# TaiseiNiman/SimpleGaussianSplat_tk71

Measured on AMD Instinct MI355X. Metric: splat-pixel pairs blended per second (grouped cumprod fwd+bwd), higher is better.
Workload: dtype f32; 1 GPU; cfg3: 1920x1080, 1000000 Gaussians, mean 80 splats/pixel (deep heavy-tailed lists); pairs_per_gpu=166335639, pixel_groups_per_gpu=2073600, bytes_per_pair=32, tiles_left_to_the_follow_up_kernel=0, world_size_checked=1, tiles_resolved_through_the_descriptor_tree=1258

## Files before the change

simplegaussiansplat_tk71_amd/csrc/gcp_bin.hip:

```cpp

#include <hip/hip_runtime.h>
#include <stdint.h>

#include "gcp_tiles.hpp"

namespace {
using namespace gcp;

constexpr int kScanChunk = 2048;

__device__ __forceinline__ int block_excl_scan_256(int v, int* s_w, int& total) {
  const int lane = threadIdx.x & 63, w = threadIdx.x >> 6;
  const int inc = wave_incl_scan_i(v);
  if (lane == 63) s_w[w] = inc;
  __syncthreads();
  int woff = 0, tot = 0;
#pragma unroll
  for (int j = 0; j < 4; ++j) { const int t = s_w[j]; if (j < w) woff += t; tot += t; }
  total = tot;
  __syncthreads();
  return woff + inc - v;
}

__global__ __launch_bounds__(256) void k_scan_reduce(const int* in, int* bsum, i64 n) {
  __shared__ int s_w[4];
  const i64 base = (i64)blockIdx.x * kScanChunk + (i64)threadIdx.x * 8;
  int s = 0;
#pragma unroll
  for (int k = 0; k < 8; ++k) if (base + k < n) s += in[base + k];
  int total;
  block_excl_scan_256(s, s_w, total);
  if (threadIdx.x == 0) bsum[blockIdx.x] = total;
}

__global__ __launch_bounds__(256) void k_scan_apply(const int* in, const int* bsum, int* out, i64 n, i64 nb) {
  __shared__ int s_w[4];
  int part = 0;
  for (i64 j = threadIdx.x; j < (i64)blockIdx.x; j += 256) part += bsum[j];
  int boff;
  block_excl_scan_256(part, s_w, boff);
  const i64 base = (i64)blockIdx.x * kScanChunk + (i64)threadIdx.x * 8;
  int v[8];
  int s = 0;
#pragma unroll
  for (int k = 0; k < 8; ++k) { v[k] = (base + k < n) ? in[base + k] : 0; s += v[k]; }
  int total;
  int ex = block_excl_scan_256(s, s_w, total) + boff;
#pragma unroll
  for (int k = 0; k < 8; ++k) { if (base + k < n) out[base + k] = ex; ex += v[k]; }
  if ((i64)blockIdx.x == nb - 1 && threadIdx.x == 0) out[n] = boff + total;
}

}

int gcp::launch_excl_scan(const int* in, int* out, i64 n, int* ws, hipStream_t stream) {
  if (n <= 0) {
    GCP_HIP(hipMemsetAsync(out, 0, sizeof(int), stream));
    return GCP_OK;
  }
  const i64 nb = (n + kScanChunk - 1) / kScanChunk;
  hipLaunchKernelGGL(k_scan_reduce, dim3((unsigned)nb), dim3(256), 0, stream, in, ws, n);
  hipLaunchKernelGGL(k_scan_apply, dim3((unsigned)nb), dim3(256), 0, stream, in, (const int*)ws, out, n, nb);
  GCP_HIP(hipGetLastError());
  return GCP_OK;
}

namespace {

__global__ __launch_bounds__(256) void k_tile_count(const int* start, const int* end, i64 n, int W, int H, int* cnt,
                                                     unsigned long long* total64) {
  __shared__ unsigned long long s_total;
  if (threadIdx.x == 0) s_total = 0;
  __syncthreads();
  unsigned long long wide = 0;
  for (i64 g = (i64)blockIdx.x * blockDim.x + threadIdx.x; g < n; g += (i64)gridDim.x * blockDim.x) {
    Box b;
    int c = 0;
    if (load_box(start, end, g, W, H, b))
      c = ((b.x1 >> kTileLog2) - (b.x0 >> kTileLog2) + 1) * ((b.y1 >> kTileLog2) - (b.y0 >> kTileLog2) + 1);
    cnt[g] = c;
    wide += (unsigned long long)c;
  }
  if (wide) atomicAdd(&s_total, wide);
  __syncthreads();
  if (threadIdx.x == 0 && s_total) atomicAdd(total64, s_total);
}

constexpr int kEmitWide = 128;
__global__ __launch_bounds__(256) void k_tile_emit(const int* start, const int* end, i64 n, int W, int H, int tiles_x,
                                                   const int* off, unsigned* key, unsigned* val, i64 capacity, int* info,
                                                   const unsigned long long* total64) {
  const i64 g = (i64)blockIdx.x * blockDim.x + threadIdx.x;
  const int lane = threadIdx.x & 63;
  bool live = g < n;
  if (info) {
    if (*total64 > 0x7fffffffull) {
      if (g == 0) { info[0] = 0; info[1] = 1; }
      return;
    }
    if (live) {
      const i64 lo = off[g], hi = off[g + 1];
      if (g == 0 && (i64)off[n] <= capacity) { info[0] = off[n]; info[1] = 0; }
      if (lo <= capacity && hi > capacity) { info[0] = (int)lo; info[1] = 1; }
      if (hi > capacity) live = false;
    }
  }
  Box b = {0, 0, -1, -1};
  if (live) live = load_box(start, end, g, W, H, b);
  const int tx0 = b.x0 >> kTileLog2, ty0 = b.y0 >> kTileLog2;
  const int ntx = live ? (b.x1 >> kTileLog2) - tx0 + 1 : 0, nty = live ? (b.y1 >> kTileLog2) - ty0 + 1 : 0;
  const int e0 = live ? off[g] : 0;
  const bool wide = ntx * nty >= kEmitWide;
  if (live && !wide) {
    int e = e0;
    for (int ty = ty0; ty < ty0 + nty; ++ty)
      for (int tx = tx0; tx < tx0 + ntx; ++tx) {
        key[e] = (unsigned)(ty * tiles_x + tx);
        val[e] = (unsigned)g;
        ++e;
      }
  }
  for (unsigned long long todo = __ballot(wide); todo; todo &= todo - 1ull) {
    const int owner = __builtin_ctzll(todo);
    const int wtx0 = __builtin_amdgcn_readlane(tx0, owner), wty0 = __builtin_amdgcn_readlane(ty0, owner);
    const int wntx = __builtin_amdgcn_readlane(ntx, owner), wcount = wntx * __builtin_amdgcn_readlane(nty, owner);
    const int we0 = __builtin_amdgcn_readlane(e0, owner);
    const unsigned wg = (unsigned)(g - lane + owner);
    for (int i = lane; i < wcount; i += 64) {
      const int ty = i / wntx, tx = i - ty * wntx;
      key[we0 + i] = (unsigned)((wty0 + ty) * tiles_x + wtx0 + tx);
      val[we0 + i] = wg;
    }
  }
}

__global__ __launch_bounds__(256) void k_sort_hist(const unsigned* key, i64 n, int shift, int* hist, int nblk, const int* n_dev,
                                                   int xcd_remap) {
  __shared__ int h[256];
  const i64 chunk = sort_chunk(blockIdx.x, nblk, xcd_remap);
  if (chunk < 0) return;
  if (n_dev) n = min(n, (i64)*n_dev);
  h[threadIdx.x] = 0;
  __syncthreads();
  const i64 base = chunk * kSortChunk;
#pragma unroll 4
  for (int i = threadIdx.x; i < kSortChunk; i += 256)
    if (base + i < n) atomicAdd(&h[(key[base + i] >> shift) & 255u], 1);
  __syncthreads();
  hist[(i64)threadIdx.x * nblk + chunk] = h[threadIdx.x];
}

__global__ __launch_bounds__(256) void k_sort_scatter(const unsigned* key, const unsigned* val, unsigned* key_out,
                                                       unsigned* val_out, i64 n, int shift, const int* hist_excl,
                                                       int nblk, const int* n_dev, int xcd_remap) {
  const i64 chunk = sort_chunk(blockIdx.x, nblk, xcd_remap);
  if (chunk < 0) return;
  if (n_dev) n = min(n, (i64)*n_dev);
  __shared__ unsigned s_key[kSortChunk];
  __shared__ unsigned s_val[kSortChunk];
  __shared__ int off[4][256];
  __shared__ int gdelta[256];
  __shared__ int s_w[4];
  const int tid = threadIdx.x, lane = tid & 63, w = tid >> 6;
  for (int d = lane; d < 256; d += 64) off[w][d] = 0;
  __syncthreads();
  const i64 bbase = chunk * kSortChunk;
  const i64 wbase = bbase + (i64)w * (kSortChunk / 4);
  constexpr int kSteps = kSortChunk / 4 / 64;
  unsigned k[kSteps], v[kSteps];
#pragma unroll
  for (int st = 0; st < kSteps; ++st) {
    const i64 i = wbase + st * 64 + lane;
    const bool valid = i < n;
    k[st] = valid ? key[i] : 0u;
    v[st] = valid ? val[i] : 0u;
    if (valid) atomicAdd(&off[w][(k[st] >> shift) & 255u], 1);
  }
  __syncthreads();
  {
    const int c0 = off[0][tid], c1 = off[1][tid], c2 = off[2][tid], c3 = off[3][tid];
    int total;
    const int lstart = block_excl_scan_256(c0 + c1 + c2 + c3, s_w, total);
    off[0][tid] = lstart;
    off[1][tid] = lstart + c0;
    off[2][tid] = lstart + c0 + c1;
    off[3][tid] = lstart + c0 + c1 + c2;
    gdelta[tid] = hist_excl[(i64)tid * nblk + chunk] - lstart;
  }
  __syncthreads();
#pragma unroll
  for (int st = 0; st < kSteps; ++st) {
    const i64 i = wbase + st * 64 + lane;
    const bool valid = i < n;
    const unsigned d = (k[st] >> shift) & 255u;
    unsigned long long peers = __ballot(valid);
#pragma unroll
    for (int b = 0; b < 8; ++b) {
      const bool bit = (d >> b) & 1u;
      const unsigned long long m = __ballot(bit);
      peers &= bit ? m : ~m;
    }
    const int rank = __builtin_popcountll(peers & ((1ull << lane) - 1ull));
    const int pos = off[w][d];
    if (valid && rank == 0) off[w][d] = pos + __builtin_popcountll(peers);
    if (valid) {
      s_key[pos + rank] = k[st];
      s_val[pos + rank] = v[st];
    }
  }
  __syncthreads();
  const int nvalid = (int)((n - bbase < kSortChunk) ? (n - bbase) : kSortChunk);
  for (int i = tid; i < nvalid; i += 256) {
    const unsigned kk = s_key[i];
    const i64 g = (i64)i + gdelta[(kk >> shift) & 255u];
    key_out[g] = kk;
    val_out[g] = s_val[i];
  }
}

__global__ void k_tile_bounds(const unsigned* key, i64 K, int n_tiles, int* tile_start, const int* n_dev) {
  if (n_dev) K = min(K, (i64)*n_dev);
  const i64 i = (i64)blockIdx.x * blockDim.x + threadIdx.x;
  if (i > K) return;
  const int prev = (i == 0) ? -1 : (int)key[i - 1];
  const int cur = (i == K) ? n_tiles : (int)key[i];
  for (int t = prev + 1; t <= cur; ++t) tile_start[t] = (int)i;
}

}

extern "C" {

int gcp_tile_grid(int32_t width, int32_t height, int32_t* tiles_x, int32_t* tiles_y) {
  if (width < 0 || height < 0 || !tiles_x || !tiles_y) return GCP_ERR_INVALID_ARGUMENT;
  const TileGrid t = tile_grid(width, height);
  *tiles_x = t.tx;
  *tiles_y = t.ty;
  return GCP_OK;
}

size_t gcp_scan_i32_workspace_bytes(int64_t n) {
  return align256((size_t)((n + kScanChunk - 1) / kScanChunk + 1) * sizeof(int));
}

int gcp_exclusive_scan_i32(const int32_t* in, int32_t* out, int64_t n, void* ws, size_t ws_bytes, void* stream) {
  if (n < 0 || !out || (n > 0 && (!in || !ws))) return GCP_ERR_INVALID_ARGUMENT;
  if (n > 0 && ws_bytes < gcp_scan_i32_workspace_bytes(n)) return GCP_ERR_WORKSPACE;
  return launch_excl_scan(in, out, n, (int*)ws, (hipStream_t)stream);
}

static int count_tiles(const int32_t* start_xy, const int32_t* end_xy, int64_t n_gauss, int32_t width, int32_t height,
                       int32_t* tile_off, unsigned long long* total64, void* ws, hipStream_t stream) {
  char* p = (char*)ws + 256;
  int* cnt = carve<int>(p, (size_t)n_gauss);
  int* sws = (int*)p;
  GCP_HIP(hipMemsetAsync(total64, 0, sizeof(unsigned long long), stream));
  const i64 count_blocks = (n_gauss + 255) / 256 < 512 ? (n_gauss + 255) / 256 : 512;
  hipLaunchKernelGGL(k_tile_count, dim3((unsigned)count_blocks), dim3(256), 0, stream, start_xy, end_xy,
                     (i64)n_gauss, width, height, cnt, total64);
  GCP_HIP(hipGetLastError());
  return launch_excl_scan(cnt, tile_off, n_gauss, sws, stream);
}

int gcp_bin_tiles_count(const int32_t* start_xy, const int32_t* end_xy, int64_t n_gauss, int32_t width,
                        int32_t height, int32_t* tile_off, int64_t* n_tile_pairs_host, void* ws,
                        size_t ws_bytes, void* stream_) {
  hipStream_t stream = (hipStream_t)stream_;
  if (n_gauss < 0 || width < 0 || height < 0 || !tile_off || !n_tile_pairs_host) return GCP_ERR_INVALID_ARGUMENT;
  *n_tile_pairs_host = 0;
  if (n_gauss == 0) {
    GCP_HIP(hipMemsetAsync(tile_off, 0, sizeof(int), stream));
    return GCP_OK;
  }
  if (!start_xy || !end_xy || !ws) return GCP_ERR_INVALID_ARGUMENT;
  const size_t need = 256 + align256((size_t)n_gauss * sizeof(int)) + gcp_scan_i32_workspace_bytes(n_gauss);
  if (ws_bytes < need) return GCP_ERR_WORKSPACE;
  unsigned long long* total64 = (unsigned long long*)ws;
  const int st = count_tiles(start_xy, end_xy, n_gauss, width, height, tile_off, total64, ws, stream);
  if (st != GCP_OK) return st;
  unsigned long long total = 0;
  GCP_HIP(hipMemcpyAsync(&total, total64, sizeof(total), hipMemcpyDeviceToHost, stream));
  GCP_HIP(hipStreamSynchronize(stream));
  if (total > 0x7fffffffull) return GCP_ERR_INVALID_ARGUMENT;
  *n_tile_pairs_host = (int64_t)total;
  return GCP_OK;
}

size_t gcp_bin_workspace_bytes(int64_t n_gauss, int64_t n_tile_pairs) {
  const int64_t k = n_tile_pairs > 0 ? n_tile_pairs : 1;
  const int64_t nblk = (k + kSortChunk - 1) / kSortChunk;
  size_t b = 0;
  b += 3 * align256((size_t)k * sizeof(unsigned));
  b += 2 * align256((size_t)(256 * nblk + 1) * sizeof(int));
  b += gcp_scan_i32_workspace_bytes(256 * nblk);
  const size_t count_need = 256 + align256((size_t)(n_gauss > 0 ? n_gauss : 1) * sizeof(int)) +
                            gcp_scan_i32_workspace_bytes(n_gauss > 0 ? n_gauss : 1);
  return (b > count_need ? b : count_need) + 512;
}

static int bin_fill(const int32_t* start_xy, const int32_t* end_xy, int64_t n_gauss, int32_t width, int32_t height,
                    const int32_t* tile_off, int64_t K, int32_t* tile_start, int32_t* tile_list, int* info,
                    const unsigned long long* total64, void* ws, hipStream_t stream) {
  const TileGrid tg = tile_grid(width, height);
  const int n_tiles = tg.tx * tg.ty;
  const i64 nblk = (K + kSortChunk - 1) / kSortChunk;
  char* p = (char*)ws;
  unsigned* keyA = carve<unsigned>(p, (size_t)K);
  unsigned* keyB = carve<unsigned>(p, (size_t)K);
  unsigned* valB = carve<unsigned>(p, (size_t)K);
  int* hist = carve<int>(p, (size_t)(256 * nblk + 1));
  int* hist_ex = carve<int>(p, (size_t)(256 * nblk + 1));
  int* sws = (int*)p;
  unsigned* valA = (unsigned*)tile_list;
  const int* n_dev = info;

  hipLaunchKernelGGL(k_tile_emit, dim3((unsigned)((n_gauss + 255) / 256)), dim3(256), 0, stream, start_xy, end_xy,
                     (i64)n_gauss, width, height, tg.tx, tile_off, keyA, valA, (i64)K, info, total64);
  GCP_HIP(hipGetLastError());
  int bits = 1;
  while ((1 << bits) < n_tiles) ++bits;
  int passes = (bits + 7) / 8;
  if (passes & 1) ++passes;
  unsigned *ks = keyA, *vs = valA, *kd = keyB, *vd = valB;
  for (int pass = 0; pass < passes; ++pass) {
    const int shift = 8 * pass;
    hipLaunchKernelGGL(k_sort_hist, dim3((unsigned)nblk), dim3(256), 0, stream, (const unsigned*)ks, K, shift, hist, (int)nblk, n_dev, 0);
    GCP_HIP(hipGetLastError());
    const int st = launch_excl_scan(hist, hist_ex, 256 * nblk, sws, stream);
    if (st != GCP_OK) return st;
    hipLaunchKernelGGL(k_sort_scatter, dim3((unsigned)nblk), dim3(256), 0, stream, (const unsigned*)ks,
                       (const unsigned*)vs, kd, vd, K, shift, (const int*)hist_ex, (int)nblk, n_dev, 0);
    GCP_HIP(hipGetLastError());
    unsigned* t;
    t = ks; ks = kd; kd = t;
    t = vs; vs = vd; vd = t;
  }
  hipLaunchKernelGGL(k_tile_bounds, dim3((unsigned)((K + 1 + 255) / 256)), dim3(256), 0, stream, ks, K, n_tiles,
                     tile_start, n_dev);
  GCP_HIP(hipGetLastError());
  return GCP_OK;
}

int gcp_bin_tiles_fill(const int32_t* start_xy, const int32_t* end_xy, int64_t n_gauss, int32_t width,
                       int32_t height, const int32_t* tile_off, int64_t n_tile_pairs, int32_t* tile_start,
                       int32_t* tile_list, void* ws, size_t ws_bytes, void* stream_) {
  hipStream_t stream = (hipStream_t)stream_;
  if (n_gauss < 0 || n_tile_pairs < 0 || width < 0 || height < 0 || !tile_start) return GCP_ERR_INVALID_ARGUMENT;
  const TileGrid tg = tile_grid(width, height);
  const int n_tiles = tg.tx * tg.ty;
  const i64 K = n_tile_pairs;
  if (K == 0) {
    GCP_HIP(hipMemsetAsync(tile_start, 0, (size_t)(n_tiles + 1) * sizeof(int), stream));
    return GCP_OK;
  }
  if (!start_xy || !end_xy || !tile_off || !tile_list || !ws) return GCP_ERR_INVALID_ARGUMENT;
  if (ws_bytes < gcp_bin_workspace_bytes(n_gauss, K)) return GCP_ERR_WORKSPACE;
  return bin_fill(start_xy, end_xy, n_gauss, width, height, tile_off, K, tile_start, tile_list, nullptr, nullptr, ws, stream);
}

int gcp_bin_tiles(const int32_t* start_xy, const int32_t* end_xy, int64_t n_gauss, int32_t width, int32_t height,
                  int64_t capacity, int32_t* tile_off, int32_t* tile_start, int32_t* tile_list, int32_t* info, void* ws,
                  size_t ws_bytes, void* stream_) {
  hipStream_t stream = (hipStream_t)stream_;
  if (n_gauss < 0 || width < 0 || height < 0 || capacity < 1 || capacity > 0x7fffffffLL || !tile_off || !tile_start || !tile_list ||
      !info || !ws)
    return GCP_ERR_INVALID_ARGUMENT;
  const TileGrid tg = tile_grid(width, height);
  const int n_tiles = tg.tx * tg.ty;
  if (n_gauss == 0) {
    GCP_HIP(hipMemsetAsync(tile_off, 0, sizeof(int), stream));
    GCP_HIP(hipMemsetAsync(tile_start, 0, (size_t)(n_tiles + 1) * sizeof(int), stream));
    GCP_HIP(hipMemsetAsync(info, 0, 2 * sizeof(int), stream));
    return GCP_OK;
  }
  if (!start_xy || !end_xy) return GCP_ERR_INVALID_ARGUMENT;
  if (ws_bytes < gcp_bin_workspace_bytes(n_gauss, capacity)) return GCP_ERR_WORKSPACE;
  unsigned long long* total64 = (unsigned long long*)((char*)ws + ((ws_bytes - 256) & ~(size_t)255));
  const int st = count_tiles(start_xy, end_xy, n_gauss, width, height, tile_off, total64, ws, stream);
  if (st != GCP_OK) return st;
  return bin_fill(start_xy, end_xy, n_gauss, width, height, tile_off, capacity, tile_start, tile_list, info, total64, ws, stream);
}

}
```

simplegaussiansplat_tk71_amd/csrc/gcp_sort.hip:

```cpp

#include <hip/hip_runtime.h>
#include <stdint.h>

#include "gcp_tiles.hpp"

namespace {
using namespace gcp;

constexpr int kBigChunk = 4096;
constexpr int kSortSub = 8;

__device__ __forceinline__ void count_runs(int* h, unsigned d, int lane) {
  const unsigned dl = (unsigned)dpp_i<0x138, 0xf>((int)0xffffffffu, (int)d);
  const bool head = (lane == 0) || (d != dl);
  const unsigned long long heads = __ballot(head);
  if (head && d < 256u) {
    const unsigned long long above = (lane == 63) ? 0ull : (heads >> (lane + 1));
    const int len = above ? (__builtin_ctzll(above) + 1) : (64 - lane);
    atomicAdd(&h[d], len);
  }
}

struct SortPass { int shift; unsigned dmask; int idw; int restore; float inv_idw; };

template <bool RECTS>
__device__ __forceinline__ unsigned load_sort_key(const unsigned* key, i64 i, int idw) {
  if (!RECTS) return key[i];
  const int2 r = reinterpret_cast<const int2*>(key)[i];
  return (unsigned)(r.y * (idw ? idw : 10000) + r.x);
}

__device__ __forceinline__ unsigned restore_key(unsigned id, int idw, float inv_idw) {
  unsigned y = (unsigned)((float)id * inv_idw);
  int x = (int)id - (int)y * idw;
  if (x < 0) { --y; x += idw; }
  else if (x >= idw) { ++y; x -= idw; }
  return y * 10000u + (unsigned)x;
}

template <bool RECTS>
__global__ __launch_bounds__(256) void k_sort_hist2(const unsigned* key, i64 n, const SortPass ps, int* hist, int nsuper, int sub, int xcd_remap,
                                                    int vec ) {
  const int shift = ps.shift;
  const unsigned dmask = ps.dmask;
  const int kmul = ps.idw ? ps.idw : 10000;
  __shared__ int h[256];
  const i64 super = sort_chunk(blockIdx.x, nsuper, xcd_remap);
  if (super < 0) return;
  const int lane = threadIdx.x & 63;
  h[threadIdx.x] = 0;
  __syncthreads();
  const i64 base = super * (i64)sub * kBigChunk;
  const i64 end = min(n, base + (i64)sub * kBigChunk);
  for (i64 p0 = base; p0 < end; p0 += 1024) {
    const i64 p = p0 + (i64)threadIdx.x * 4;
    unsigned k4[4];
    if (vec && p + 3 < end) {
      if (RECTS) {
        const int4 a = *reinterpret_cast<const int4*>(reinterpret_cast<const int2*>(key) + p);
        const int4 b = *reinterpret_cast<const int4*>(reinterpret_cast<const int2*>(key) + p + 2);
        k4[0] = (unsigned)(a.y * kmul + a.x); k4[1] = (unsigned)(a.w * kmul + a.z);
        k4[2] = (unsigned)(b.y * kmul + b.x); k4[3] = (unsigned)(b.w * kmul + b.z);
      } else {
        const uint4 a = *reinterpret_cast<const uint4*>(key + p);
        k4[0] = a.x; k4[1] = a.y; k4[2] = a.z; k4[3] = a.w;
      }
#pragma unroll
      for (int j = 0; j < 4; ++j) k4[j] = (k4[j] >> shift) & dmask;
    } else {
#pragma unroll
      for (int j = 0; j < 4; ++j) k4[j] = (p + j < end) ? ((load_sort_key<RECTS>(key, p + j, ps.idw) >> shift) & dmask) : 256u;
    }
#pragma unroll
    for (int j = 0; j < 4; ++j) count_runs(h, k4[j], lane);
  }
  __syncthreads();
  hist[(i64)threadIdx.x * nsuper + super] = h[threadIdx.x];
}

__device__ __forceinline__ void digit_peers(unsigned d, unsigned long long valid, unsigned& lo, unsigned& hi) {
  unsigned acc_lo = 0u, acc_hi = 0u;
#pragma unroll
  for (int b = 0; b < 8; ++b) {
    const int sb = ((int)(d << (31 - b))) >> 31;
    const unsigned long long m = __ballot(sb != 0);
    acc_lo |= (unsigned)m ^ (unsigned)sb;
    acc_hi |= (unsigned)(m >> 32) ^ (unsigned)sb;
  }
  lo = (unsigned)valid & ~acc_lo;
  hi = (unsigned)(valid >> 32) & ~acc_hi;
}

constexpr int kSortWaves = kBigChunk / 512;

template <bool FIRST, bool RECTS>
__global__ __launch_bounds__(64 * kSortWaves) void k_sort_scatter2(const unsigned* key, const unsigned* val, unsigned* key_out,
                                                                    unsigned* val_out, i64 n, const SortPass ps, const int* hist_excl,
                                                                    int nsuper, int sub, int xcd_remap) {
  const i64 super = sort_chunk(blockIdx.x, nsuper, xcd_remap);
  if (super < 0) return;
  const int shift = ps.shift;
  const unsigned dmask = ps.dmask;
  __shared__ unsigned s_key[kBigChunk];
  __shared__ unsigned s_val[kBigChunk];
  __shared__ int off[kSortWaves][256];
  __shared__ int gdelta[256];
  __shared__ int gbase[256];
  __shared__ int s_w[4];
  const int tid = threadIdx.x, lane = tid & 63, w = tid >> 6;
  constexpr int kThreadsS = 64 * kSortWaves;
  constexpr int kWaveKeys = kBigChunk / kSortWaves;
  constexpr int kSteps = kWaveKeys / 64;
  const i64 sbase = super * (i64)sub * kBigChunk;
  const int nsub = (int)min((i64)sub, (n - sbase + kBigChunk - 1) / kBigChunk);
  if (tid < 256) gbase[tid] = hist_excl[(i64)tid * nsuper + super];
  for (int c = 0; c < nsub; ++c) {
    const i64 bbase = sbase + (i64)c * kBigChunk;
    const i64 wbase = bbase + (i64)w * kWaveKeys;
    unsigned k[kSteps], v[kSteps];
#pragma unroll
    for (int st = 0; st < kSteps; ++st) {
      const i64 i = wbase + st * 64 + lane;
      const bool valid = i < n;
      k[st] = valid ? load_sort_key<RECTS>(key, i, ps.idw) : 0u;
      v[st] = FIRST ? (unsigned)i : (valid ? val[i] : 0u);
    }
    for (int d = lane; d < 256; d += 64) off[w][d] = 0;
    __syncthreads();
    int slot[kSteps];
#pragma unroll
    for (int st = 0; st < kSteps; ++st) {
      const bool valid = wbase + st * 64 + lane < n;
      const unsigned d = (k[st] >> shift) & dmask;
      unsigned plo, phi;
      digit_peers(d, __ballot(valid), plo, phi);
      const int rank = (int)__builtin_amdgcn_mbcnt_hi(phi, __builtin_amdgcn_mbcnt_lo(plo, 0u));
      const int cnt = __builtin_popcount(plo) + __builtin_popcount(phi);
      int before = 0;
      if (valid && rank == 0) before = atomicAdd(&off[w][d], cnt);
      const int leader = plo ? __builtin_ctz(plo) : (32 + __builtin_ctz(phi | 0x80000000u));
      before = __builtin_amdgcn_ds_bpermute(leader << 2, before);
      slot[st] = before + rank;
    }
    __syncthreads();
    {
      int cw[kSortWaves], sum = 0;
      if (tid < 256) {
#pragma unroll
        for (int j = 0; j < kSortWaves; ++j) { cw[j] = off[j][tid]; sum += cw[j]; }
      }
      const int inc = wave_incl_scan_i(sum);
      if (lane == 63 && w < 4) s_w[w] = inc;
      __syncthreads();
      if (tid < 256) {
        int run = inc - sum;
#pragma unroll
        for (int j = 0; j < 4; ++j)
          if (j < w) run += s_w[j];
        const int gb = gbase[tid];
        gdelta[tid] = gb - run;
        gbase[tid] = gb + sum;
#pragma unroll
        for (int j = 0; j < kSortWaves; ++j) { off[j][tid] = run; run += cw[j]; }
      }
    }
    __syncthreads();
#pragma unroll
    for (int st = 0; st < kSteps; ++st) {
      if (wbase + st * 64 + lane < n) {
        const int pos = off[w][(k[st] >> shift) & dmask] + slot[st];
        s_key[pos] = k[st];
        s_val[pos] = v[st];
      }
    }
    __syncthreads();
    const int nvalid = (int)((n - bbase < kBigChunk) ? (n - bbase) : kBigChunk);
    for (int i = tid; i < nvalid; i += kThreadsS) {
      const unsigned kk = s_key[i];
      const i64 g = (i64)i + gdelta[(kk >> shift) & dmask];
      if ((unsigned long long)g < (unsigned long long)n) {
        key_out[g] = ps.restore ? restore_key(kk, ps.idw, ps.inv_idw) : kk;
        val_out[g] = s_val[i];
      }
    }
  }
}

__global__ void k_gather_f32(const float* __restrict__ src, const int* __restrict__ index, float* __restrict__ dst, i64 n) {
  const i64 i = (i64)blockIdx.x * blockDim.x + threadIdx.x;
  if (i < n) dst[i] = src[index[i]];
}
__global__ void k_unsort_finish(const float* __restrict__ incl, const float* __restrict__ sorted_x,
                                const int* __restrict__ index, float* __restrict__ full, unsigned char* __restrict__ keep,
                                i64 n, int mode) {
  const i64 i = (i64)blockIdx.x * blockDim.x + threadIdx.x;
  if (i >= n) return;
  const float v = incl[i], x = sorted_x[i];
  const int o = index[i];
  full[o] = mode == 0 ? v / x : v - x;
  keep[o] = v != 0.0f ? 1 : 0;
}

__global__ __launch_bounds__(256) void k_rects_key_range(const int* rects, i64 n, int* out ) {
  __shared__ int s_mx[4], s_mn[4];
  int mx = 0, mn = 0x7fffffff;
  for (i64 i = (i64)blockIdx.x * 256 + threadIdx.x; i < n; i += (i64)gridDim.x * 256) {
    const int2 r = reinterpret_cast<const int2*>(rects)[i];
    mx = max(mx, r.y * 10000 + r.x);
    mn = min(mn, min(r.x, r.y));
  }
  for (int o = 32; o > 0; o >>= 1) {
    mx = max(mx, __shfl_xor(mx, o));
    mn = min(mn, __shfl_xor(mn, o));
  }
  if ((threadIdx.x & 63) == 0) { s_mx[threadIdx.x >> 6] = mx; s_mn[threadIdx.x >> 6] = mn; }
  __syncthreads();
  if (threadIdx.x == 0) {
    atomicMax(out, max(max(s_mx[0], s_mx[1]), max(s_mx[2], s_mx[3])));
    atomicMin(out + 1, min(min(s_mn[0], s_mn[1]), min(s_mn[2], s_mn[3])));
  }
}

}

extern "C" {

int gcp_gather_f32(const float* src, const int32_t* index, float* dst, int64_t n, void* stream_) {
  if (n < 0) return GCP_ERR_INVALID_ARGUMENT;
  if (n == 0) return GCP_OK;
  if (!src || !index || !dst) return GCP_ERR_INVALID_ARGUMENT;
  hipLaunchKernelGGL(k_gather_f32, dim3((unsigned)((n + 255) / 256)), dim3(256), 0, (hipStream_t)stream_, src, index, dst, (i64)n);
  GCP_HIP(hipGetLastError());
  return GCP_OK;
}

int gcp_unsort_finish(const float* inclusive, const float* sorted_x, const int32_t* index, float* full, uint8_t* keep,
                      int64_t n, int32_t mode, void* stream_) {
  if (n < 0 || (mode != 0 && mode != 1)) return GCP_ERR_INVALID_ARGUMENT;
  if (n == 0) return GCP_OK;
  if (!inclusive || !sorted_x || !index || !full || !keep) return GCP_ERR_INVALID_ARGUMENT;
  hipLaunchKernelGGL(k_unsort_finish, dim3((unsigned)((n + 255) / 256)), dim3(256), 0, (hipStream_t)stream_, inclusive, sorted_x,
                     index, full, keep, (i64)n, mode);
  GCP_HIP(hipGetLastError());
  return GCP_OK;
}

size_t gcp_sort_workspace_bytes(int64_t n) {
  const int64_t m = n > 0 ? n : 1;
  const int64_t nblk = (m + kSortChunk - 1) / kSortChunk;
  size_t b = 2 * align256((size_t)m * sizeof(unsigned));
  b += 2 * align256((size_t)(256 * nblk + 1) * sizeof(int));
  b += gcp_scan_i32_workspace_bytes(256 * nblk);
  return b;
}

static int sort_impl(const unsigned* keys_in, bool rects, int64_t n, int32_t key_bits, int32_t id_width, uint32_t* keys_out,
                     int32_t* index_out, void* ws, size_t ws_bytes, hipStream_t stream) {
  if (n < 0 || n > 0x7fffffffLL || key_bits < 1 || key_bits > 32 || id_width < 0 || (id_width && (!rects || key_bits > 24)))
    return GCP_ERR_INVALID_ARGUMENT;
  if (n == 0) return GCP_OK;
  if (!keys_in || !keys_out || !index_out || !ws) return GCP_ERR_INVALID_ARGUMENT;
  if (ws_bytes < gcp_sort_workspace_bytes(n)) return GCP_ERR_WORKSPACE;
  constexpr int xcd_remap = 1;
  const i64 nblk = (n + kBigChunk - 1) / kBigChunk;
  int sub = (int)(nblk / 2048);
  sub = sub < 1 ? 1 : (sub > kSortSub ? kSortSub : sub);
  const i64 nsuper = (nblk + sub - 1) / sub;
  const dim3 grid(sort_grid(nsuper, xcd_remap)), block(256);
  char* p = (char*)ws;
  unsigned* keyY = carve<unsigned>(p, (size_t)n);
  unsigned* valY = carve<unsigned>(p, (size_t)n);
  int* hist = carve<int>(p, (size_t)(256 * nblk + 1));
  int* hist_ex = carve<int>(p, (size_t)(256 * nblk + 1));
  int* sws = (int*)p;
  unsigned* keyX = keys_out;
  unsigned* valX = (unsigned*)index_out;
  const int passes = (key_bits + 7) / 8;
  const int width = (key_bits + passes - 1) / passes;
  const unsigned* ks = keys_in;
  const unsigned* vs = nullptr;
  for (int pass = 0; pass < passes; ++pass) {
    const bool to_x = ((passes - 1 - pass) & 1) == 0;
    unsigned* kd = to_x ? keyX : keyY;
    unsigned* vd = to_x ? valX : valY;
    SortPass ps;
    ps.shift = width * pass;
    ps.dmask = (1u << width) - 1u;
    ps.idw = id_width;
    ps.restore = (id_width && pass == passes - 1) ? 1 : 0;
    ps.inv_idw = id_width ? 1.0f / (float)id_width : 0.0f;
    const bool src_rects = pass == 0 && rects;
    const int vec = (((uintptr_t)ks & 15u) == 0) ? 1 : 0;
    if (src_rects) hipLaunchKernelGGL((k_sort_hist2<true>), grid, block, 0, stream, ks, (i64)n, ps, hist, (int)nsuper, sub, xcd_remap, vec);
    else hipLaunchKernelGGL((k_sort_hist2<false>), grid, block, 0, stream, ks, (i64)n, ps, hist, (int)nsuper, sub, xcd_remap, vec);
    GCP_HIP(hipGetLastError());
    const int st = launch_excl_scan(hist, hist_ex, 256 * nsuper, sws, stream);
    if (st != GCP_OK) return st;
    const dim3 sblock(64 * kSortWaves);
    if (src_rects)
      hipLaunchKernelGGL((k_sort_scatter2<true, true>), grid, sblock, 0, stream, ks, vs, kd, vd, (i64)n, ps, (const int*)hist_ex,
                         (int)nsuper, sub, xcd_remap);
    else if (pass == 0)
      hipLaunchKernelGGL((k_sort_scatter2<true, false>), grid, sblock, 0, stream, ks, vs, kd, vd, (i64)n, ps, (const int*)hist_ex,
                         (int)nsuper, sub, xcd_remap);
    else
      hipLaunchKernelGGL((k_sort_scatter2<false, false>), grid, sblock, 0, stream, ks, vs, kd, vd, (i64)n, ps, (const int*)hist_ex,
                         (int)nsuper, sub, xcd_remap);
    GCP_HIP(hipGetLastError());
    ks = kd;
    vs = vd;
  }
  return GCP_OK;
}

int gcp_sort_pairs_u32(const uint32_t* keys_in, int64_t n, int32_t key_bits, uint32_t* keys_out, int32_t* index_out,
                       void* ws, size_t ws_bytes, void* stream_) {
  return sort_impl(keys_in, false, n, key_bits, 0, keys_out, index_out, ws, ws_bytes, (hipStream_t)stream_);
}

int gcp_sort_rects(const int32_t* rects_xy, int64_t n, int32_t key_bits, int32_t id_width, uint32_t* keys_out, int32_t* index_out,
                   void* ws, size_t ws_bytes, void* stream_) {
  return sort_impl((const unsigned*)rects_xy, true, n, key_bits, id_width, keys_out, index_out, ws, ws_bytes, (hipStream_t)stream_);
}

int gcp_rects_key_range(const int32_t* rects_xy, int64_t n, int32_t* out_dev, void* stream_) {
  hipStream_t stream = (hipStream_t)stream_;
  if (n < 0 || !out_dev) return GCP_ERR_INVALID_ARGUMENT;
  GCP_HIP(hipMemsetD32Async((hipDeviceptr_t)out_dev, 0, 1, stream));
  GCP_HIP(hipMemsetD32Async((hipDeviceptr_t)(out_dev + 1), 0x7fffffff, 1, stream));
  if (n == 0) return GCP_OK;
  if (!rects_xy) return GCP_ERR_INVALID_ARGUMENT;
  i64 blocks = (n + 4095) / 4096;
  if (blocks > 2048) blocks = 2048;
  hipLaunchKernelGGL(k_rects_key_range, dim3((unsigned)blocks), dim3(256), 0, stream, rects_xy, (i64)n, out_dev);
  GCP_HIP(hipGetLastError());
  return GCP_OK;
}

}
```

simplegaussiansplat_tk71_amd/csrc/gcp_tiles.hpp:

```cpp
#pragma once
#include "gcp_device.hpp"
#include "grouped_cumprod_hip.h"

namespace gcp {

constexpr int kTileLog2 = 4;
constexpr int kTile = 1 << kTileLog2;
constexpr int kStage = 256;
constexpr int kSortChunk = 4096;
constexpr int kDropTileLog2 = 12;
constexpr int kCompactTile = 1 << kDropTileLog2;

struct TileGrid { int tx, ty; };
inline TileGrid tile_grid(int W, int H) { return {(W + 1 + kTile - 1) / kTile, (H + 1 + kTile - 1) / kTile}; }

struct Box { int x0, y0, x1, y1; };
__device__ __forceinline__ bool load_box(const int* start, const int* end, i64 g, int W, int H, Box& b) {
  b.x0 = max(start[2 * g], 0);
  b.y0 = max(start[2 * g + 1], 0);
  b.x1 = min(end[2 * g], W);
  b.y1 = min(end[2 * g + 1], H);
  return b.x1 >= b.x0 && b.y1 >= b.y0;
}

__device__ __forceinline__ i64 sort_chunk(i64 b, i64 nblk, int xcd_remap) {
  if (!xcd_remap) return b < nblk ? b : -1;
  const i64 per = (nblk + 7) >> 3;
  const i64 c = (b & 7) * per + (b >> 3);
  return ((b >> 3) < per && c < nblk) ? c : -1;
}
inline unsigned sort_grid(i64 nblk, int xcd_remap) { return (unsigned)(xcd_remap ? ((nblk + 7) >> 3) * 8 : nblk); }

__device__ __forceinline__ unsigned long long uniform64(unsigned long long v) {
  return ((unsigned long long)(unsigned)__builtin_amdgcn_readfirstlane((int)(v >> 32)) << 32) |
         (unsigned)__builtin_amdgcn_readfirstlane((int)v);
}

int launch_excl_scan(const int* in, int* out, i64 n, int* ws, hipStream_t stream);

}

namespace {

struct BlendArgs {
  const int* start;
  const int* end;
  const float* mean;
  const float* vinv;
  const float* opacity;
  const float* l_d;
  const int* tile_start;
  const unsigned* tile_list;
  int W, H, tiles_x;
};

inline int make_args(BlendArgs& a, const int32_t* start_xy, const int32_t* end_xy, const float* mean_xy,
                     const float* vinv, const float* opacity, const float* l_d, int32_t width, int32_t height,
                     const int32_t* tile_start, const int32_t* tile_list) {
  if (width < 0 || height < 0 || !tile_start) return GCP_ERR_INVALID_ARGUMENT;
  a.start = start_xy; a.end = end_xy; a.mean = mean_xy; a.vinv = vinv; a.opacity = opacity; a.l_d = l_d;
  a.tile_start = tile_start; a.tile_list = (const unsigned*)tile_list;
  a.W = width; a.H = height; a.tiles_x = gcp::tile_grid(width, height).tx;
  return GCP_OK;
}

}
```

Before: 216.9 billion pairs/s.

## Replace global histogram scan with per-digit row scans and fuse tile count reduce

The radix sort no longer runs a two-kernel exclusive scan over the whole 256×nblk histogram. A single kernel now scans each digit row independently and records a per-digit total. The scatter kernels then scan those 256 totals on the fly to rebuild global bucket bases. The tile-count kernel also writes per-block sums itself, so the separate scan-reduce launch is dropped and only the scan-apply kernel follows. This removes kernel launches and a pass over the histogram, but adds a small redundant scan in every scatter block and serialises each digit row's scan inside one block.

```diff
diff --git a/simplegaussiansplat_tk71_amd/csrc/gcp_bin.hip b/simplegaussiansplat_tk71_amd/csrc/gcp_bin.hip
--- a/simplegaussiansplat_tk71_amd/csrc/gcp_bin.hip
+++ b/simplegaussiansplat_tk71_amd/csrc/gcp_bin.hip
@@ -51,6 +51,32 @@
   if ((i64)blockIdx.x == nb - 1 && threadIdx.x == 0) out[n] = boff + total;
 }
 
+__global__ __launch_bounds__(256) void k_digit_offsets(const int* hist, int* row_excl, int* tot, i64 nblk) {
+  __shared__ int s_w[4];
+  const int* row = hist + (i64)blockIdx.x * nblk;
+  int* out = row_excl + (i64)blockIdx.x * nblk;
+  int carry = 0;
+  for (i64 b0 = 0; b0 < nblk; b0 += 1024) {
+    const i64 b = b0 + (i64)threadIdx.x * 4;
+    int v[4];
+    int s = 0;
+#pragma unroll
+    for (int k = 0; k < 4; ++k) { v[k] = (b + k < nblk) ? row[b + k] : 0; s += v[k]; }
+    int total;
+    int ex = block_excl_scan_256(s, s_w, total) + carry;
+#pragma unroll
+    for (int k = 0; k < 4; ++k) { if (b + k < nblk) out[b + k] = ex; ex += v[k]; }
+    carry += total;
+  }
+  if (threadIdx.x == 0) tot[blockIdx.x] = carry;
+}
+
+}
+
+int gcp::launch_digit_offsets(const int* hist, int* row_excl, int* tot, int ndig, i64 nblk, hipStream_t stream) {
+  hipLaunchKernelGGL(k_digit_offsets, dim3((unsigned)ndig), dim3(256), 0, stream, hist, row_excl, tot, nblk);
+  GCP_HIP(hipGetLastError());
+  return GCP_OK;
 }
 
 int gcp::launch_excl_scan(const int* in, int* out, i64 n, int* ws, hipStream_t stream) {
@@ -67,23 +93,31 @@
 
 namespace {
 
-__global__ __launch_bounds__(256) void k_tile_count(const int* start, const int* end, i64 n, int W, int H, int* cnt,
+__global__ __launch_bounds__(256) void k_tile_count(const int* start, const int* end, i64 n, int W, int H, int* cnt, int* bsum,
                                                      unsigned long long* total64) {
   __shared__ unsigned long long s_total;
   if (threadIdx.x == 0) s_total = 0;
   __syncthreads();
   unsigned long long wide = 0;
-  for (i64 g = (i64)blockIdx.x * blockDim.x + threadIdx.x; g < n; g += (i64)gridDim.x * blockDim.x) {
-    Box b;
-    int c = 0;
-    if (load_box(start, end, g, W, H, b))
-      c = ((b.x1 >> kTileLog2) - (b.x0 >> kTileLog2) + 1) * ((b.y1 >> kTileLog2) - (b.y0 >> kTileLog2) + 1);
-    cnt[g] = c;
-    wide += (unsigned long long)c;
+  const i64 base = (i64)blockIdx.x * kScanChunk;
+#pragma unroll
+  for (int k = 0; k < kScanChunk / 256; ++k) {
+    const i64 g = base + k * 256 + threadIdx.x;
+    if (g < n) {
+      Box b;
+      int c = 0;
+      if (load_box(start, end, g, W, H, b))
+        c = ((b.x1 >> kTileLog2) - (b.x0 >> kTileLog2) + 1) * ((b.y1 >> kTileLog2) - (b.y0 >> kTileLog2) + 1);
+      cnt[g] = c;
+      wide += (unsigned long long)c;
+    }
   }
   if (wide) atomicAdd(&s_total, wide);
   __syncthreads();
-  if (threadIdx.x == 0 && s_total) atomicAdd(total64, s_total);
+  if (threadIdx.x == 0) {
+    bsum[blockIdx.x] = (int)s_total;
+    if (s_total) atomicAdd(total64, s_total);
+  }
 }
 
 constexpr int kEmitWide = 128;
@@ -151,11 +185,13 @@
 }
 
 __global__ __launch_bounds__(256) void k_sort_scatter(const unsigned* key, const unsigned* val, unsigned* key_out,
-                                                       unsigned* val_out, i64 n, int shift, const int* hist_excl,
-                                                       int nblk, const int* n_dev, int xcd_remap) {
+                                                       unsigned* val_out, i64 n, int shift, const int* row_excl,
+                                                       const int* tot, int nblk, const int* n_dev, int xcd_remap) {
   const i64 chunk = sort_chunk(blockIdx.x, nblk, xcd_remap);
   if (chunk < 0) return;
   if (n_dev) n = min(n, (i64)*n_dev);
+  const int row_before = row_excl[(i64)threadIdx.x * nblk + chunk];
+  const int digit_total = tot[threadIdx.x];
   __shared__ unsigned s_key[kSortChunk];
   __shared__ unsigned s_val[kSortChunk];
   __shared__ int off[4][256];
@@ -185,7 +221,8 @@
     off[1][tid] = lstart + c0;
     off[2][tid] = lstart + c0 + c1;
     off[3][tid] = lstart + c0 + c1 + c2;
-    gdelta[tid] = hist_excl[(i64)tid * nblk + chunk] - lstart;
+    const int digit_first = block_excl_scan_256(digit_total, s_w, total);
+    gdelta[tid] = digit_first + row_before - lstart;
   }
   __syncthreads();
 #pragma unroll
@@ -255,11 +292,12 @@
   int* cnt = carve<int>(p, (size_t)n_gauss);
   int* sws = (int*)p;
   GCP_HIP(hipMemsetAsync(total64, 0, sizeof(unsigned long long), stream));
-  const i64 count_blocks = (n_gauss + 255) / 256 < 512 ? (n_gauss + 255) / 256 : 512;
-  hipLaunchKernelGGL(k_tile_count, dim3((unsigned)count_blocks), dim3(256), 0, stream, start_xy, end_xy,
-                     (i64)n_gauss, width, height, cnt, total64);
+  const i64 nb = (n_gauss + kScanChunk - 1) / kScanChunk;
+  hipLaunchKernelGGL(k_tile_count, dim3((unsigned)nb), dim3(256), 0, stream, start_xy, end_xy, (i64)n_gauss, width, height, cnt, sws,
+                     total64);
+  hipLaunchKernelGGL(k_scan_apply, dim3((unsigned)nb), dim3(256), 0, stream, (const int*)cnt, (const int*)sws, tile_off, (i64)n_gauss, nb);
   GCP_HIP(hipGetLastError());
-  return launch_excl_scan(cnt, tile_off, n_gauss, sws, stream);
+  return GCP_OK;
 }
 
 int gcp_bin_tiles_count(const int32_t* start_xy, const int32_t* end_xy, int64_t n_gauss, int32_t width,
@@ -292,7 +330,7 @@
   size_t b = 0;
   b += 3 * align256((size_t)k * sizeof(unsigned));
   b += 2 * align256((size_t)(256 * nblk + 1) * sizeof(int));
-  b += gcp_scan_i32_workspace_bytes(256 * nblk);
+  b += align256(256 * sizeof(int));
   const size_t count_need = 256 + align256((size_t)(n_gauss > 0 ? n_gauss : 1) * sizeof(int)) +
                             gcp_scan_i32_workspace_bytes(n_gauss > 0 ? n_gauss : 1);
   return (b > count_need ? b : count_need) + 512;
@@ -310,7 +348,7 @@
   unsigned* valB = carve<unsigned>(p, (size_t)K);
   int* hist = carve<int>(p, (size_t)(256 * nblk + 1));
   int* hist_ex = carve<int>(p, (size_t)(256 * nblk + 1));
-  int* sws = (int*)p;
+  int* dtot = carve<int>(p, 256);
   unsigned* valA = (unsigned*)tile_list;
   const int* n_dev = info;
 
@@ -326,10 +364,10 @@
     const int shift = 8 * pass;
     hipLaunchKernelGGL(k_sort_hist, dim3((unsigned)nblk), dim3(256), 0, stream, (const unsigned*)ks, K, shift, hist, (int)nblk, n_dev, 0);
     GCP_HIP(hipGetLastError());
-    const int st = launch_excl_scan(hist, hist_ex, 256 * nblk, sws, stream);
+    const int st = launch_digit_offsets(hist, hist_ex, dtot, 256, nblk, stream);
     if (st != GCP_OK) return st;
     hipLaunchKernelGGL(k_sort_scatter, dim3((unsigned)nblk), dim3(256), 0, stream, (const unsigned*)ks,
-                       (const unsigned*)vs, kd, vd, K, shift, (const int*)hist_ex, (int)nblk, n_dev, 0);
+                       (const unsigned*)vs, kd, vd, K, shift, (const int*)hist_ex, (const int*)dtot, (int)nblk, n_dev, 0);
     GCP_HIP(hipGetLastError());
     unsigned* t;
     t = ks; ks = kd; kd = t;
diff --git a/simplegaussiansplat_tk71_amd/csrc/gcp_sort.hip b/simplegaussiansplat_tk71_amd/csrc/gcp_sort.hip
--- a/simplegaussiansplat_tk71_amd/csrc/gcp_sort.hip
+++ b/simplegaussiansplat_tk71_amd/csrc/gcp_sort.hip
@@ -75,7 +75,7 @@
     for (int j = 0; j < 4; ++j) count_runs(h, k4[j], lane);
   }
   __syncthreads();
-  hist[(i64)threadIdx.x * nsuper + super] = h[threadIdx.x];
+  if (threadIdx.x <= dmask) hist[(i64)threadIdx.x * nsuper + super] = h[threadIdx.x];
 }
 
 __device__ __forceinline__ void digit_peers(unsigned d, unsigned long long valid, unsigned& lo, unsigned& hi) {
@@ -95,8 +95,8 @@
 
 template <bool FIRST, bool RECTS>
 __global__ __launch_bounds__(64 * kSortWaves) void k_sort_scatter2(const unsigned* key, const unsigned* val, unsigned* key_out,
-                                                                    unsigned* val_out, i64 n, const SortPass ps, const int* hist_excl,
-                                                                    int nsuper, int sub, int xcd_remap) {
+                                                                    unsigned* val_out, i64 n, const SortPass ps, const int* row_excl,
+                                                                    const int* tot, int nsuper, int sub, int xcd_remap) {
   const i64 super = sort_chunk(blockIdx.x, nsuper, xcd_remap);
   if (super < 0) return;
   const int shift = ps.shift;
@@ -113,7 +113,21 @@
   constexpr int kSteps = kWaveKeys / 64;
   const i64 sbase = super * (i64)sub * kBigChunk;
   const int nsub = (int)min((i64)sub, (n - sbase + kBigChunk - 1) / kBigChunk);
-  if (tid < 256) gbase[tid] = hist_excl[(i64)tid * nsuper + super];
+  {
+    const bool row = tid <= (int)dmask;
+    const int t = row ? tot[tid] : 0;
+    const int before = row ? row_excl[(i64)tid * nsuper + super] : 0;
+    const int inc = wave_incl_scan_i(t);
+    if (lane == 63 && w < 4) s_w[w] = inc;
+    __syncthreads();
+    if (tid < 256) {
+      int first = inc - t;
+#pragma unroll
+      for (int j = 0; j < 4; ++j)
+        if (j < w) first += s_w[j];
+      gbase[tid] = first + before;
+    }
+  }
   for (int c = 0; c < nsub; ++c) {
     const i64 bbase = sbase + (i64)c * kBigChunk;
     const i64 wbase = bbase + (i64)w * kWaveKeys;
@@ -250,7 +264,7 @@
   const int64_t nblk = (m + kSortChunk - 1) / kSortChunk;
   size_t b = 2 * align256((size_t)m * sizeof(unsigned));
   b += 2 * align256((size_t)(256 * nblk + 1) * sizeof(int));
-  b += gcp_scan_i32_workspace_bytes(256 * nblk);
+  b += align256(256 * sizeof(int));
   return b;
 }
 
@@ -270,13 +284,13 @@
   char* p = (char*)ws;
   unsigned* keyY = carve<unsigned>(p, (size_t)n);
   unsigned* valY = carve<unsigned>(p, (size_t)n);
+  const int passes = (key_bits + 7) / 8;
+  const int width = (key_bits + passes - 1) / passes;
   int* hist = carve<int>(p, (size_t)(256 * nblk + 1));
   int* hist_ex = carve<int>(p, (size_t)(256 * nblk + 1));
-  int* sws = (int*)p;
+  int* dtot = carve<int>(p, 256);
   unsigned* keyX = keys_out;
   unsigned* valX = (unsigned*)index_out;
-  const int passes = (key_bits + 7) / 8;
-  const int width = (key_bits + passes - 1) / passes;
   const unsigned* ks = keys_in;
   const unsigned* vs = nullptr;
   for (int pass = 0; pass < passes; ++pass) {
@@ -294,18 +308,18 @@
     if (src_rects) hipLaunchKernelGGL((k_sort_hist2<true>), grid, block, 0, stream, ks, (i64)n, ps, hist, (int)nsuper, sub, xcd_remap, vec);
     else hipLaunchKernelGGL((k_sort_hist2<false>), grid, block, 0, stream, ks, (i64)n, ps, hist, (int)nsuper, sub, xcd_remap, vec);
     GCP_HIP(hipGetLastError());
-    const int st = launch_excl_scan(hist, hist_ex, 256 * nsuper, sws, stream);
+    const int st = launch_digit_offsets(hist, hist_ex, dtot, 1 << width, nsuper, stream);
     if (st != GCP_OK) return st;
     const dim3 sblock(64 * kSortWaves);
     if (src_rects)
       hipLaunchKernelGGL((k_sort_scatter2<true, true>), grid, sblock, 0, stream, ks, vs, kd, vd, (i64)n, ps, (const int*)hist_ex,
-                         (int)nsuper, sub, xcd_remap);
+                         (const int*)dtot, (int)nsuper, sub, xcd_remap);
     else if (pass == 0)
       hipLaunchKernelGGL((k_sort_scatter2<true, false>), grid, sblock, 0, stream, ks, vs, kd, vd, (i64)n, ps, (const int*)hist_ex,
-                         (int)nsuper, sub, xcd_remap);
+                         (const int*)dtot, (int)nsuper, sub, xcd_remap);
     else
       hipLaunchKernelGGL((k_sort_scatter2<false, false>), grid, sblock, 0, stream, ks, vs, kd, vd, (i64)n, ps, (const int*)hist_ex,
-                         (int)nsuper, sub, xcd_remap);
+                         (const int*)dtot, (int)nsuper, sub, xcd_remap);
     GCP_HIP(hipGetLastError());
     ks = kd;
     vs = vd;
diff --git a/simplegaussiansplat_tk71_amd/csrc/gcp_tiles.hpp b/simplegaussiansplat_tk71_amd/csrc/gcp_tiles.hpp
--- a/simplegaussiansplat_tk71_amd/csrc/gcp_tiles.hpp
+++ b/simplegaussiansplat_tk71_amd/csrc/gcp_tiles.hpp
@@ -38,6 +38,8 @@
 
 int launch_excl_scan(const int* in, int* out, i64 n, int* ws, hipStream_t stream);
 
+int launch_digit_offsets(const int* hist, int* row_excl, int* tot, int ndig, i64 nblk, hipStream_t stream);
+
 }
 
 namespace {
```

Measured after the change: 217.9 billion pairs/s, median of 3. About the same (+0.4%).
